# author-hidden-name/GAN-segmentation

Measured on AMD Instinct MI355X. Metric: synthetic (image,mask) pairs/sec, FFHQ-1024 StyleGAN+decoder, higher is better.
Workload: dtype f32; 1 GPU; stylegan-ffhq 1024^2 synthesis + 2-class decoder, batch=8 per GPU, fp32 (BASELINE.json configs[1]); synthetic weights/latents/noise; (img u8, mask u8) resident on rank 0; global_batch=8, parallelism=dp1, gather=none, backend=none, graph=eager (GSA_GRAPH=0)

## Files before the change

gan-segmentation_amd/csrc/gsa_api.cpp:

```cpp
#include <hip/hip_runtime.h>

#include <cmath>
#include <cstdarg>
#include <cstdio>
#include <cstdlib>
#include <cstring>
#include <map>
#include <string>
#include <vector>

#include "../../include/gsa.h"
#include "gsa_kernels.h"
#include "gsa_pack.h"

using namespace gsa;

namespace {

constexpr int kMaxLevels = 12;
thread_local std::string g_create_error;

struct HostTensor {
    std::vector<float> data;
    std::vector<int64_t> dims;
// ... 213 lines not shown
}

bool known_generator_name(const gsa_ctx* c, const char* name) {
    int R = 0, k = 0, i = 0;
    char tail[64], t2[64];
    if (!strcmp(name, "constant_tensor") || !strcmp(name, "latent_avg") || !strcmp(name, "truncation_psi")) return true;
    if (sscanf(name, "mp_dense_%d_%63s", &i, tail) == 2)
        return i >= 0 && i < 8 && (!strcmp(tail, "weight") || !strcmp(tail, "bias") || !strcmp(tail, "std"));
    if (sscanf(name, "%d_%63s", &R, tail) != 2) return false;
    int r = 0;
    while ((1 << r) < R) ++r;
    if ((1 << r) != R || r < 2 || r > c->gc.max_res_log2) return false;
    if (!strcmp(tail, "conv_1_weight") || !strcmp(tail, "conv_1_std")) return r > 2 && r < 7;
    if (!strcmp(tail, "deconv_1_weight") || !strcmp(tail, "deconv_1_std")) return r >= 7;
    if (!strcmp(tail, "blur_1_w_kernel")) return r > 2;
    if (!strcmp(tail, "conv_2_weight") || !strcmp(tail, "conv_2_std")) return true;
    if (!strcmp(tail, "conv_to_rgb_weight") || !strcmp(tail, "conv_to_rgb_bias") || !strcmp(tail, "conv_to_rgb_std"))
        return r == c->gc.max_res_log2;
    if (sscanf(tail, "noise_%d_%63s", &k, t2) == 2) return (k == 1 || k == 2) && !strcmp(t2, "scale_factors");
    if (sscanf(tail, "bias_%d_%63s", &k, t2) == 2) return (k == 1 || k == 2) && !strcmp(t2, "bias");
    if (sscanf(tail, "adain_%d_%63s", &k, t2) == 2)
        return (k == 1 || k == 2) &&
               (!strcmp(t2, "dense_affine_weight") || !strcmp(t2, "dense_affine_bias") || !strcmp(t2, "dense_affine_std") ||
                !strcmp(t2, "norm_gamma") || !strcmp(t2, "norm_beta"));
    return false;
}

int set_param(gsa_ctx* c, std::map<std::string, HostTensor>& m, const char* name, const float* data, int ndim,
              const int64_t* dims) {
    if (!name || !data || ndim < 0 || ndim > 8) return fail(c, GSA_ERR_INVALID, "bad parameter tensor %s", name ? name : "(null)");
    HostTensor t;
    size_t cnt = 1;
    for (int i = 0; i < ndim; ++i) {
        if (dims[i] < 0) return fail(c, GSA_ERR_INVALID, "negative dimension in %s", name);
        t.dims.push_back(dims[i]);
        cnt *= (size_t)dims[i];
    }
    t.data.assign(data, data + cnt);
    m[name] = std::move(t);
    return GSA_OK;
}


struct Launch {
    gsa_ctx* c;
    hipStream_t s;
    const char* label;
    double flops, bytes, alg;
    std::string entry_layer;
    hipEvent_t a = nullptr;
    Launch(gsa_ctx* ctx, hipStream_t st, const char* layer, double flops_, double bytes_, double alg_ = -1.0)
        : c(ctx), s(st), label(layer), flops(flops_), bytes(bytes_), alg(alg_ < 0 ? flops_ : alg_) {
        (void)take_launch_record();
        if (!c->prof) return;
        if (c->prof > 1 && layer) entry_layer = layer;
        if (c->bf16 && layer && strncmp(layer, "g.mapping", 9) && strncmp(layer, "g.styles", 8) && !strstr(layer, "finalize")) bytes *= 0.5;
        a = event();
        (void)hipEventRecord(a, s);
    }
    hipEvent_t event() {
        if (c->event_pool.empty()) {
            hipEvent_t e = nullptr;
            (void)hipEventCreate(&e);
            return e;
        }
        hipEvent_t e = c->event_pool.back();
        c->event_pool.pop_back();
        return e;
    }
    ~Launch() {
        const LaunchRecord r = take_launch_record();
#ifdef GSA_STAMP
        const std::string kname_s = r.count == 1 ? kernel_name(r.kern) : std::string();
        const char* kname = kname_s.c_str();
        if (c->stamps && label && (strstr(kname, "conv") || strstr(kname, "subpixel"))) {
            (void)hipStreamSynchronize(s);
            unsigned long long h[16];
            (void)hipMemcpy(h, c->stamps, sizeof h, hipMemcpyDeviceToHost);
            (void)hipMemset(c->stamps, 0, sizeof h);
            if (h[15] && strstr(kname, "_ws")) {
                const double w = (double)h[15];
                fprintf(stderr, "STAMPWS %-24s %-16s waves %6llu  mfma: work %9.0f barrier %9.0f | mem: write %9.0f load %9.0f epi %9.0f barrier %9.0f\n",
                        kname, label, h[15], h[0] / w, h[1] / w, h[2] / w, h[3] / w, h[4] / w, h[5] / w);
            } else if (h[15] && h[8]) {
                const double w = (double)h[12];
                fprintf(stderr, "STAMPDB %-70s %-14s waves %6llu items/wave %5.1f | per item: write %6.0f load %6.0f (epi-loads %5.0f index %5.0f bulk %5.0f) mfma %6.0f epi %6.0f barrier %6.0f\n",
                        kname, label, h[15], h[12] / (double)h[15], h[6] / w, h[7] / w, h[0] / w, h[1] / w, h[2] / w, h[8] / w, h[9] / w, h[10] / w);
                if (strstr(kname, "subpixel"))
                    fprintf(stderr, "STAMPSW %-14s barrier by wave: %6.0f %6.0f %6.0f %6.0f | write wave0 %6.0f wave3 %6.0f\n", label, 4 * h[0] / w, 4 * h[1] / w, 4 * h[2] / w, 4 * h[3] / w, 4 * h[4] / w, 4 * h[5] / w);
            } else if (h[15]) {
                const double w = (double)h[15];
                fprintf(stderr, "STAMP %-40s %-16s waves %8llu  load %7.0f  write %6.0f  bar %6.0f  blocks %8.0f  epi %7.0f\n", kname,
                        label, h[15], h[0] / w, h[1] / w, h[2] / w, h[3] / w, h[4] / w);
            }
        }
#endif
        if (!a) return;
        if (r.count != 1) {
            c->event_pool.push_back(a);
            if (r.count > 1) ++c->prof_multi;
            return;
        }
        int entry = -1;
        for (size_t i = 0; i < c->prof_entries.size() && entry < 0; ++i)
            if (c->prof_entries[i].kern == r.kern && c->prof_entries[i].layer == entry_layer) entry = (int)i;
        if (entry < 0) {
            ProfEntry e;
            e.kern = r.kern;
            e.layer = entry_layer;
            c->prof_entries.push_back(e);
            entry = (int)c->prof_entries.size() - 1;
        }
        ProfEntry& e = c->prof_entries[entry];
        e.flops += flops;
        e.alg_flops += alg;
        e.bytes += bytes;
        e.launches += 1;
        hipEvent_t b = event();
        (void)hipEventRecord(b, s);
        c->prof_events.push_back(ProfEvent{a, b, entry});
    }
};

}


extern "C" {

#define GSA_STR2(x) #x
#define GSA_STR(x) GSA_STR2(x)
const char* gsa_version(void) {
#ifndef GSA_EXPERIMENTS
#define GSA_EXPERIMENTS 0
#endif
    return "gsa-hip 0.5"
#if GSA_EXPERIMENTS
           "+experiments"
#endif
           " (gfx950, v_mfma_f32_16x16x4_f32 implicit-GEMM convs; built with hipcc = clang " __clang_version__
           ", HIP " GSA_STR(HIP_VERSION_MAJOR) "." GSA_STR(HIP_VERSION_MINOR) "." GSA_STR(HIP_VERSION_PATCH) ")";
}

int gsa_create(int device, gsa_ctx** out) {
    if (!out) return fail(nullptr, GSA_ERR_INVALID, "gsa_create: out is null");
    int count = 0;
    hipError_t e = hipGetDeviceCount(&count);
    if (e != hipSuccess || count <= 0)
        return fail(nullptr, GSA_ERR_HIP, "no HIP device available (%s)", e == hipSuccess ? "device count is 0" : hipGetErrorString(e));
    if (device < 0 || device >= count) return fail(nullptr, GSA_ERR_INVALID, "device %d out of range (%d devices)", device, count);
    e = hipSetDevice(device);
    if (e != hipSuccess) return fail(nullptr, GSA_ERR_HIP, "hipSetDevice(%d): %s", device, hipGetErrorString(e));
    gsa_ctx* c = new gsa_ctx();
    c->device = device;
    e = hipStreamCreateWithFlags(&c->side, hipStreamNonBlocking);
    for (int i = 0; e == hipSuccess && i < kMaxLevels; ++i) e = hipEventCreateWithFlags(&c->ev_level[i], hipEventDisableTiming);
    if (e == hipSuccess) e = hipEventCreateWithFlags(&c->ev_fork, hipEventDisableTiming);
    if (e == hipSuccess) e = hipEventCreateWithFlags(&c->ev_join, hipEventDisableTiming);
    if (e != hipSuccess) {
        const int rc = fail(nullptr, GSA_ERR_HIP, "creating the side stream: %s", hipGetErrorString(e));
        delete c;
        return rc;
    }
    if (e == hipSuccess) e = hipMalloc((void**)&c->zeros, 256);
    if (e == hipSuccess) e = hipMemset(c->zeros, 0, 256);
    if (e != hipSuccess) {
        const int rc = fail(nullptr, GSA_ERR_HIP, "allocating the zero page: %s", hipGetErrorString(e));
// ... 866 lines not shown
```

gan-segmentation_amd/csrc/gsa_kernels.hip:

```cpp
#include "gsa_kernels.h"
#include "gsa_dev.h"

#include <cxxabi.h>

#include <cstdio>
#include <cstdlib>
#include <cstring>
#include <mutex>
#include <vector>

#ifndef GSA_MFMA_PRIO
#define GSA_MFMA_PRIO 2
#endif
#ifndef GSA_OPERAND_PIPELINE
#define GSA_OPERAND_PIPELINE 1
#endif
#ifndef GSA_NO_XCD_REMAP
#define GSA_NO_XCD_REMAP 0
#endif
#ifndef GSA_POST_OCC
#define GSA_POST_OCC 2
#endif
#ifndef GSA_WINO_SOA
#define GSA_WINO_SOA 0
// ... 569 lines not shown
            TSUM(s0, k1, ka); TSUM(s1, ka, kb); TSUM(s2, kb, k2);
            mfma_item(it & 1, cb);
            TICK(k3);
            if (cb == nblk - 1) {
                epilogue(tc);
                if (stats_direct && (it + 1 >= total_items || tr.n != tc.n || tr.g != tc.g)) flush_stats(tc);
            }
            TICK(k4);
            write_aff_item(it & 1);
            __syncthreads();
            TICK(k5);
            TSUM(sw, k0, k1); TSUM(sl, k1, k2); TSUM(sm, k2, k3); TSUM(se, k3, k4); TSUM(sb, k4, k5);
            tc = tr; cb = cbr; tr = t2; cbr = cb2;
        }
        TFLUSH(6, sw); TFLUSH(7, sl); TFLUSH(8, sm); TFLUSH(9, se); TFLUSH(10, sb);
        TFLUSH(0, s0); TFLUSH(1, s1); TFLUSH(2, s2);
        TFLUSH(12, (unsigned long long)total_items); TFLUSH(15, 1ull);
        return;
    }

    WorkTile tc = decode(w_begin);
    TilePixel tp[AIT], tpn[AIT];
    tile_pixels(tc, tp);
    load_item(tc, 0, tp);
    int n_aff = tc.n;
    if (has_aff) {
        write_aff();
        __syncthreads();
    }
#ifdef GSA_STAMP
    asm volatile("s_waitcnt vmcnt(0)" ::: "memory");
#endif
    STAMP(1);
    write_item(0, tp, is_edge(tc));
    STAMP(2);
    __syncthreads();
    STAMP(3);

    int w = w_begin, cb = 0;
    while (true) {
        int w2 = w, cb2 = cb + 1;
        if (cb2 == nblk) { cb2 = 0; w2 = w + 1; }
        const bool has_next = w2 < w_end;
        if (!has_next) { w2 = w; cb2 = cb; }
        WorkTile tn = tc;
        if (w2 != w) {
            tn = advance(tc);
            tile_pixels(tn, tpn);
        } else {
#pragma unroll
            for (int it = 0; it < AIT; ++it) tpn[it] = tp[it];
        }
        load_item(tn, cb2, tpn);
        __builtin_amdgcn_sched_barrier(0);
        mfma_item(0);
        __builtin_amdgcn_sched_barrier(0);

        if (cb == nblk - 1) { epilogue_loads(tc); epilogue(tc); }
        if (!has_next) break;
        __syncthreads();
        if (has_aff && tn.n != n_aff) {
            write_aff();
            n_aff = tn.n;
            __syncthreads();
        }
#ifdef GSA_DBG_HOOKS
        if (!(p.dbg & 8))
#endif
        write_item(cb2, tpn, is_edge(tn));
        __syncthreads();
        tc = tn; w = w2; cb = cb2;
#pragma unroll
        for (int it = 0; it < AIT; ++it) tp[it] = tpn[it];
    }
    STAMP(4);
#ifdef GSA_STAMP
    asm volatile("s_waitcnt vmcnt(0)" ::: "memory");
#endif
    STAMP(5);
    STAMP_FLUSH(5);
}

__device__ __forceinline__ void finalize_one(const FinalizeParams& p, int n, int c, unsigned long long I1, unsigned long long I2);
template <int TH, int EPI, bool BF, int PS>
__global__ __launch_bounds__(256 * PS) void conv3x3_ksplit(ConvParams p) {
    constexpr int NTHR = 256 * PS, MT = (TH / 4) * (TH / 4), PW = TH / 4;
    constexpr int MTW = MT / PS;
    constexpr int LH = TH + 2, LW = TH + 2, NPX = LH * LW;
    constexpr int PX = BF ? 8 : 16, TS = BF ? 128 : 256, KQ = BF ? 2 : 4;
    constexpr int RS = LW * PX + (BF ? 4 : 8);
    constexpr int SEG = 9 * TS, IMG = LH * RS;
    constexpr int NB4 = 4 * SEG / 4, BIT = (NB4 + NTHR - 1) / NTHR;
    constexpr int QPT = PS == 1 ? 4 : 1;
    static_assert(PS == 1 || (PS == 2 && MT == 4 && 4 * NPX <= NTHR), "patch split: 8x8 tiles, one staged unit per thread");
    static_assert(NPX <= NTHR, "one staged pixel per thread and block");
    extern __shared__ __attribute__((aligned(16))) float smem[];
    float* sA = smem;
    float* sB = sA + 2 * 4 * IMG;
    f32x4* sAff = reinterpret_cast<f32x4*>(sB + 2 * 4 * SEG);
    f32x4* sP = sAff + 2 * 4 * 16;
    unsigned long long (*sfin)[16] = reinterpret_cast<unsigned long long (*)[16]>(sP + 4 * MT * 64);
    unsigned& sfin_cnt = *reinterpret_cast<unsigned*>(sfin + 2);
    if (EPI == EPI_SYNTH && p.fin_aff != nullptr && threadIdx.x < 33) {
        if (threadIdx.x < 32) sfin[threadIdx.x >> 4][threadIdx.x & 15] = 0ull; else sfin_cnt = 0u;
    }

    const int tid = threadIdx.x, lane = tid & 63;
    const int wave = __builtin_amdgcn_readfirstlane(tid >> 6);
    const int quarter = wave & 3, half = wave >> 2;
    const int i16 = lane & 15, kq = lane >> 4;
    const int tx = blockIdx.x % p.tiles_x, ty = blockIdx.x / p.tiles_x;
    const int g = blockIdx.y, n = blockIdx.z;
    const int y0 = ty * TH, x0 = tx * TH;
    const int nblk = p.C0 >> 4, nq = nblk >> 2;
    const bool has_aff = p.aff0 != nullptr;

    const int sq0 = PS == 1 ? 0 : tid / NPX;
    TilePixel tp;
    {
        const int st = PS == 1 ? tid : tid % NPX;
        const int ly = st / LW, lx = st % LW;
        const int gy = y0 + ly - 1, gx = x0 + lx - 1;
        const bool stage = PS == 1 ? tid < NPX : tid < 4 * NPX;
        const bool inside = stage && (unsigned)gy < (unsigned)p.H && (unsigned)gx < (unsigned)p.W;
        tp.lds = stage ? ly * RS + lx * PX : -1;
        tp.pix = inside ? (n * p.Hs + (gy >> p.up)) * p.Ws + (gx >> p.up) : -1;
    }
    int abase[MTW];
#pragma unroll
    for (int m = 0; m < MTW; ++m) {
        const int mt = half * MTW + m;
        abase[m] = ((mt / PW) * 4 + (i16 >> 2)) * RS + ((mt % PW) * 4 + (i16 & 3)) * PX + kq * KQ;
    }
    const int bbase = (kq * 16 + i16) * KQ;

    f32x4 acc[MTW];
#pragma unroll
    for (int m = 0; m < MTW; ++m) acc[m] = f32x4{0.f, 0.f, 0.f, 0.f};
    f32x4 ra[QPT][4], rb[BIT], rf;
    rf = f32x4{0.f, 0.f, 0.f, 0.f};
    const float* wgrp = p.wpk + (size_t)g * nblk * SEG;
    auto load_item = [&](int it) {
#pragma unroll
        for (int u = 0; u < QPT; ++u) load_pixel<BF>(ra[u], p.src0, p.C0, ((min(sq0, 3) + u) * nq + it) * 16, tp);
#pragma unroll
        for (int j = 0; j < BIT; ++j) {
            const int i = min(tid + j * NTHR, NB4 - 1);
            const int q = i / (SEG / 4), r = i % (SEG / 4);
            rb[j] = reinterpret_cast<const f32x4*>(wgrp + (size_t)(q * nq + it) * SEG)[r];
        }
        if (has_aff && tid < 64) rf = reinterpret_cast<const f32x4*>(p.aff0 + (size_t)n * p.C0 + ((tid >> 4) * nq + it) * 16)[tid & 15];
    };
    auto write_aff = [&](int buf) {
        if (has_aff && tid < 64) sAff[buf * 64 + tid] = rf;
    };
    auto write_item = [&](int buf) {
#pragma unroll
        for (int u = 0; u < QPT; ++u) {
            const int q = min(sq0, 3) + u;
            float* a_img = sA + (buf * 4 + q) * IMG;
            const float4* tab = reinterpret_cast<const float4*>(sAff) + (buf * 4 + q) * 16;
            if (has_aff) store_pixel<true, BF, true>(a_img, ra[u], tab, tp);
            else store_pixel<false, BF, true>(a_img, ra[u], tab, tp);
        }
#pragma unroll
        for (int j = 0; j < BIT; ++j) reinterpret_cast<f32x4*>(sB + buf * 4 * SEG)[min(tid + j * NTHR, NB4 - 1)] = rb[j];
    };
    auto mfma_item = [&](int buf) {
        const float* a_img = sA + (buf * 4 + quarter) * IMG;
        const float* b_img = sB + (buf * 4 + quarter) * SEG + bbase;
#pragma unroll
        for (int tap = 0; tap < 9; ++tap) {
            const int toff = (tap / 3) * RS + (tap % 3) * PX;
            if constexpr (BF) {
                const s16x4 b = *reinterpret_cast<const s16x4*>(b_img + tap * TS);
#pragma unroll
                for (int m = 0; m < MTW; ++m)
                    acc[m] = __builtin_amdgcn_mfma_f32_16x16x16bf16_1k(*reinterpret_cast<const s16x4*>(a_img + abase[m] + toff), b, acc[m], 0, 0, 0);
            } else {
                f32x4 a[MTW];
#pragma unroll
                for (int m = 0; m < MTW; ++m) a[m] = *reinterpret_cast<const f32x4*>(a_img + abase[m] + toff);
                const f32x4 b = *reinterpret_cast<const f32x4*>(b_img + tap * 256);
#pragma unroll
                for (int cg = 0; cg < 4; ++cg)
#pragma unroll
                    for (int m = 0; m < MTW; ++m) acc[m] = __builtin_amdgcn_mfma_f32_16x16x4f32(a[m][cg], b[cg], acc[m], 0, 0, 0);
            }
        }
    };

    load_item(0);
    write_aff(0);
    __syncthreads();
    write_item(0);
    load_item(min(1, nq - 1));
    write_aff(1);
    __syncthreads();
    unsigned long long k0 = 0, k1 = 0, k2 = 0, k3 = 0, k4 = 0, sw = 0, sl = 0, sm = 0, sb = 0;
    (void)k0; (void)k1; (void)k2; (void)k3; (void)k4; (void)sw; (void)sl; (void)sm; (void)sb;
    for (int it = 0; it < nq; ++it) {
        TICK(k0);
        if (it + 1 < nq) write_item((it + 1) & 1);
        TICK(k1);
        load_item(min(it + 2, nq - 1));
        TICK(k2);
        mfma_item(it & 1);
        TICK(k3);
        write_aff(it & 1);
        __syncthreads();
        TICK(k4);
        TSUM(sw, k0, k1); TSUM(sl, k1, k2); TSUM(sm, k2, k3); TSUM(sb, k3, k4);
    }
    TFLUSH(6, sw); TFLUSH(7, sl); TFLUSH(8, sm); TFLUSH(10, sb); TFLUSH(12, (unsigned long long)nq); TFLUSH(15, 1ull);
#pragma unroll
    for (int m = 0; m < MTW; ++m) sP[(quarter * MT + half * MTW + m) * 64 + lane] = acc[m];
    __syncthreads();
    if (wave >= MT) return;
    const int mt = wave;
    const f32x4 s01 = sP[(0 * MT + mt) * 64 + lane] + sP[(1 * MT + mt) * 64 + lane];
    const f32x4 s23 = sP[(2 * MT + mt) * 64 + lane] + sP[(3 * MT + mt) * 64 + lane];
    const f32x4 tot = s01 + s23;
    float v[4] = {tot[0], tot[1], tot[2], tot[3]};
    const int pr = mt / PW, pc = mt % PW, prow = lane >> 4;
    const int co = g * 16 + i16;
    const int y = y0 + pr * 4 + prow, xb = x0 + pc * 4;
    const int xj = lane & 3, cq4 = ((lane >> 2) & 3) * 4;
    if (EPI == EPI_SYNTH) {
        const float4 nz = *reinterpret_cast<const float4*>(p.noise + ((size_t)(n * p.H + y) * p.W + xb));
        const float nzv[4] = {nz.x, nz.y, nz.z, nz.w};
        const float e0 = p.nscale[co], e1 = p.nbias[co];
#pragma unroll
        for (int r = 0; r < 4; ++r) {
            const float t = e0 * nzv[r];
            v[r] = lrelu((v[r] + t) + e1);
        }
        const float sq = (v[0] + v[1]) + (v[2] + v[3]);
        const float qq = (v[0] * v[0] + v[1] * v[1]) + (v[2] * v[2] + v[3] * v[3]);
        unsigned long long I1 = to_fixed(sq, kStatScale1), I2 = to_fixed_sq(qq, stat_s2(p.H * p.W));
        I1 += shfl_xor_u64(I1, 16); I2 += shfl_xor_u64(I2, 16);
        I1 += shfl_xor_u64(I1, 32); I2 += shfl_xor_u64(I2, 32);
        if (p.fin_aff != nullptr) {
            if (lane < 16) { atomicAdd(&sfin[0][i16], I1); atomicAdd(&sfin[1][i16], I2); }
            __threadfence_block();
            unsigned arrived = 0;
            if (lane == 0) arrived = atomicAdd(&sfin_cnt, 1u);
            arrived = __shfl(arrived, 0);
            if (arrived == (unsigned)MT - 1u && lane < 16) {
                __threadfence_block();
                FinalizeParams f{};
                f.HW = p.H * p.W; f.C = p.Cout; f.style = p.fin_style; f.style_stride = p.fin_style_stride;
                f.gamma = p.fin_gamma; f.beta = p.fin_beta; f.aff = p.fin_aff; f.flags = p.fin_flags;
                finalize_one(f, n, co, atomicAdd(&sfin[0][i16], 0ull), atomicAdd(&sfin[1][i16], 0ull));
            }
        } else if (lane < 16) {
            StatPart sp; sp.s1 = I1; sp.s2 = I2;
            p.partials[((size_t)n * p.prow + blockIdx.x * MT + mt) * p.Cout + co] = sp;
        }
    }
    if (EPI == EPI_DEC) {
        const float e2 = p.bn_s[co], e3 = p.bn_beta[co];
#pragma unroll
        for (int r = 0; r < 4; ++r) {
            v[r] = lrelu(fmaf(v[r], e2, e3));
        }
    }
    f32x4 vt = quad_transpose(v[0], v[1], v[2], v[3], xj);
    if (EPI == EPI_DEC && p.resid != nullptr) {
        const int ru = p.resid_up;
        const size_t rpix = (size_t)(n * (p.H >> ru) + (y >> ru)) * (p.W >> ru) + ((xb + xj) >> ru);
        const int cch = g * 16;
        const bool second = p.resid1 != nullptr && cch >= p.res_c0;
        const int rcs = second ? p.Cout - p.res_c0 : (p.resid1 ? p.res_c0 : p.Cout);
        const f32x4 rr = act_load4<BF>((second ? p.resid1 : p.resid), rpix * rcs + (second ? cch - p.res_c0 : cch) + cq4);
#pragma unroll
        for (int r = 0; r < 4; ++r) vt[r] = rr[r] + vt[r];
    }
    act_store4<BF>(p.out, ((size_t)(n * p.H + y) * p.W + xb + xj) * p.Cout + g * 16 + cq4, vt);
}

template <int EPI, int NT, bool CHUNK, bool AFF, int GW = 1, int TW = 1>
__global__ __launch_bounds__(256 * GW * TW, NT == 1 ? 2 / TW : 1) void conv3x3_wino(ConvParams p) {
    static_assert(TW == 1 || (TW == 2 && GW == 1 && NT == 1), "two tiles per workgroup: one channel group, 16 output channels");
    constexpr int NTHR = 256 * GW * TW, LH = 18, LW = 16 * TW + 2, RS = LW * 16 + 4;
    constexpr int SEG = 16 * 256;
    constexpr int NB4 = SEG / 4, BIT = NT * NB4 / 256;
    constexpr int NCH = CHUNK ? (LH * LW * 4 + NTHR - 1) / NTHR : (LH * LW + NTHR - 1) / NTHR;
    constexpr int RW = CHUNK ? 1 : 4;
    extern __shared__ __attribute__((aligned(16))) float smem[];
    const int nblk = p.C0 >> 4;
    const bool wres = p.w_resident != 0;
    float* sA = smem;
    float* sB = sA + 2 * LH * RS;
    f32x4* sAff = reinterpret_cast<f32x4*>(sB + (wres ? nblk : 2) * GW * NT * SEG);

    const int tid = threadIdx.x, lane = tid & 63;
    const int wave8 = __builtin_amdgcn_readfirstlane(tid >> 6);
    const int wave = wave8 & 3;
    const int gsel = TW == 2 ? 0 : wave8 >> 2;
    const int tsel = TW == 2 ? wave8 >> 2 : 0;
    const int tid8 = tid & 255;
    const int i16 = lane & 15, kq = lane >> 4;
    int g, w_begin, w_end;
    if (p.group_minor) {
        const int b = blockIdx.x, j = b >> 3;
        g = (j % p.groups) * GW + gsel;
        w_begin = (j / p.groups) * 8 + (b & 7);
        w_end = w_begin + 1;
    } else {
        g = (int)blockIdx.y * GW + gsel;
        const int chunk = (p.total_tiles + (int)gridDim.x - 1) / (int)gridDim.x;
        w_begin = xcd_block(blockIdx.x, gridDim.x) * chunk;
        w_end = min(p.total_tiles, w_begin + chunk);
    }
    if (w_begin >= w_end) return;
    struct Tile { int n, y0, x0, row; };
    auto advance = [&](const Tile& t) {
        Tile u = t;
        u.x0 += 16 * TW; u.row += 1;
        if (u.x0 == p.W) { u.x0 = 0; u.y0 += 16; if (u.y0 == p.H) { u.y0 = 0; u.row = 0; u.n += 1; } }
        return u;
    };
    auto is_edge = [&](const Tile& t) { return t.y0 == 0 || t.x0 == 0 || t.y0 + 16 == p.H || t.x0 + 16 * TW == p.W; };
    const int part = tid & 3;
    int t_ly[NCH], t_lx[NCH], t_lds[NCH];
#pragma unroll
    for (int k = 0; k < NCH; ++k) {
        const int idx = CHUNK ? (tid + k * NTHR) >> 2 : tid + k * NTHR;
        t_ly[k] = idx / LW - 1; t_lx[k] = idx % LW - 1;
        t_lds[k] = idx < LH * LW ? (idx / LW) * RS + (idx % LW) * 16 + (CHUNK ? part * 4 : 0) : -1;
    }
    int t_rel[NCH];
#pragma unroll
    for (int k = 0; k < NCH; ++k) t_rel[k] = t_lds[k] >= 0 ? t_ly[k] * p.W + t_lx[k] : 0;
    auto tile_chunks = [&](const Tile& t, Chunk (&tp)[NCH]) {
        const int base = (t.n * p.H + t.y0) * p.W + t.x0;
        if (t.y0 == 0 || t.x0 == 0 || t.y0 + 16 == p.H || t.x0 + 16 * TW == p.W) {
#pragma unroll
            for (int k = 0; k < NCH; ++k) {
                const int gy = t.y0 + t_ly[k], gx = t.x0 + t_lx[k];
                const bool inside = t_lds[k] >= 0 && (unsigned)gy < (unsigned)p.H && (unsigned)gx < (unsigned)p.W;
                tp[k].lds = t_lds[k];
                tp[k].pix = inside ? base + t_rel[k] : -1;
            }
        } else {
#pragma unroll
            for (int k = 0; k < NCH; ++k) { tp[k].lds = t_lds[k]; tp[k].pix = base + t_rel[k]; }
        }
    };
    const int wty = ((i16 >> 3) & 1) * 2 + ((i16 >> 1) & 1), wtx = ((i16 >> 2) & 1) * 2 + (i16 & 1);
    const int pbase = ((wave >> 1) * 8 + 2 * wty) * RS + (tsel * 16 + (wave & 1) * 8 + 2 * wtx) * 16 + kq * 4;
    const int bbase = (kq * 16 + i16) * 4;

    f32x4 acc[16][NT];
#pragma unroll
    for (int f = 0; f < 16; ++f)
#pragma unroll
        for (int nt = 0; nt < NT; ++nt) acc[f][nt] = f32x4{0.f, 0.f, 0.f, 0.f};

    constexpr bool has_aff = AFF;
    constexpr bool kSoA = GSA_WINO_SOA != 0;
// ... 2417 lines not shown
    return enabled;
}

struct ConvGeom { int th, wm, wn, nt; };
static const ConvGeom kGeom4[] = {{4, 1, 4, 1}, {4, 1, 2, 1}, {4, 1, 1, 1}};
static const ConvGeom kGeom8[] = {{8, 4, 1, 4}, {8, 4, 1, 2}, {8, 4, 1, 1}};
static const ConvGeom kGeom16[] = {{16, 4, 1, 4}, {16, 4, 1, 2}, {16, 4, 1, 1}, {8, 4, 1, 4}, {8, 4, 1, 2}, {8, 4, 1, 1}};

static ConvGeom pick_geom(int H, int W, int Cout, int n) {
    const ConvGeom* cand = H == 4 ? kGeom4 : (H == 8 ? kGeom8 : kGeom16);
    const int ncand = H == 4 ? 3 : (H == 8 ? 3 : 6);
    ConvGeom best = cand[ncand - 1];
    long best_wgs = -1;
    for (int i = 0; i < ncand; ++i) {
        const ConvGeom& c = cand[i];
        const int ct = 16 * c.nt * c.wn;
        if (Cout % ct) continue;
        const long wgs = (long)(H / c.th) * (W / c.th) * (Cout / ct) * n;
        if (wgs >= 512) return c;
        if (wgs > best_wgs) { best_wgs = wgs; best = c; }
    }
    return best;
}

int conv_stat_rows(int H, int W, int Cout, int n) {
    const ConvGeom c = pick_geom(H, W, Cout, n);
    return (H / c.th) * (W / c.th) * c.wm;
}

int post_prow(int H, int W, int C) { return (H * (W / 4) * (C / 4) + 255) / 256; }

template <int TH, int TW, int WM, int WN, int NT, int EPI, bool SC, bool BF>
static hipError_t launch_conv_t(const ConvParams& p, int n, hipStream_t s) {
    constexpr int Q = NT * WN, COUT_T = 16 * Q;
    constexpr int TS = BF ? 128 : 256;
    constexpr int RS = (TW + 2) * (BF ? 8 : 16) + (BF ? 4 : 8);
    constexpr int NBUF = (Q <= 2 && !SC && (TH == 16 || GSA_DB_SMALL)) ? 2 : 1;
    const int nblk_all = (p.C0 + p.C1) / 16;
    static const bool wres_enabled = env_int("GSA_WRES", 1) != 0;
    const bool wres = wres_enabled && NBUF == 2 && p.Cout == COUT_T && (size_t)nblk_all * Q * 9 * TS * sizeof(float) <= 40 * 1024;
    if (NBUF == 1 && p.C0 > 512 && p.aff0) return hipErrorInvalidValue;
    const int wslots = wres ? nblk_all * Q * 9 * TS : NBUF * Q * 9 * TS;
    const size_t lds = sizeof(float) * (NBUF * (TH + 2) * RS + wslots + (SC ? Q * TS : 0)) +
                       (p.aff0 ? sizeof(float4) * (NBUF == 2 ? 32 : p.C0) : 0);
    constexpr auto kern = conv3x3_mfma<TH, TW, WM, WN, NT, EPI, SC, BF>;
    int wgs_per_cu = 0;
    if (hipError_t e = kernel_occupancy<kern>(p.device, 64 * WM * WN, lds, &wgs_per_cu)) return e;
    const int num_cus = device_cus(p.device);
    ConvParams q = p;
    q.w_resident = wres ? 1 : 0;
    q.tiles_x = p.W / TW;
    q.tiles_y = p.H / TH;
    q.groups = p.Cout / COUT_T;
    q.prow = q.tiles_x * q.tiles_y * WM;
    q.total_tiles = q.tiles_x * q.tiles_y * q.groups * n;
    const bool persistent = (p.C0 + p.C1) <= 32 && q.total_tiles > num_cus * wgs_per_cu;
    const int grid = persistent ? num_cus * wgs_per_cu : q.total_tiles;
    static const bool direct_enabled = env_int("GSA_STATS_DIRECT", 1) != 0;
    q.stats_direct = (direct_enabled && EPI == EPI_SYNTH && NBUF == 2 && persistent && p.partials != nullptr) ? 1 : 0;
    if (q.stats_direct) q.prow = kDirectRows;
    if (p.stat_rows_host) *p.stat_rows_host = q.prow;
    return launch<kern>(p.device, dim3(grid), dim3(64 * WM * WN), lds, s, q);
}

template <int TH, int TW, int WM, int WN, int NT>
static hipError_t launch_conv_g(const ConvParams& p, int epi, bool sc, int n, hipStream_t s) {
    if (sc && epi != EPI_DEC) return hipErrorInvalidValue;
#define GSA_EPI(BF) \
    if (sc) return launch_conv_t<TH, TW, WM, WN, NT, EPI_DEC, true, BF>(p, n, s); \
    if (epi == EPI_RAW) return launch_conv_t<TH, TW, WM, WN, NT, EPI_RAW, false, BF>(p, n, s); \
    if (epi == EPI_SYNTH) return launch_conv_t<TH, TW, WM, WN, NT, EPI_SYNTH, false, BF>(p, n, s); \
    if (epi == EPI_DEC) return launch_conv_t<TH, TW, WM, WN, NT, EPI_DEC, false, BF>(p, n, s); \
    return hipErrorInvalidValue;
    if (p.bf16) { GSA_EPI(true) }
    GSA_EPI(false)
#undef GSA_EPI
}

static bool ksplit_rule(const ConvParams& p, bool sc) {
    static const bool enabled = env_int("GSA_KSPLIT", 1) != 0;
    return enabled && !sc && p.src1 == nullptr && p.C1 == 0 && p.C0 >= 64 && p.C0 % 64 == 0 && (p.H <= 8 || (p.H <= 32 && p.Cout <= 32)) && p.H == p.W && p.Cout % 16 == 0;
}

template <int TH, int EPI, bool BF, int PS>
static hipError_t launch_ksplit_t(const ConvParams& p, int n, hipStream_t s) {
    constexpr int MT = (TH / 4) * (TH / 4), PX = BF ? 8 : 16, TS = BF ? 128 : 256;
    constexpr int RS = (TH + 2) * PX + (BF ? 4 : 8), IMG = (TH + 2) * RS, SEG = 9 * TS;
    const size_t lds = sizeof(float) * (2 * 4 * IMG + 2 * 4 * SEG) + sizeof(float4) * (2 * 4 * 16 + 4 * MT * 64) + 2 * 16 * sizeof(unsigned long long) + 16;
    ConvParams q = p;
    q.tiles_x = p.W / TH;
    q.tiles_y = p.H / TH;
    q.groups = p.Cout / 16;
    q.prow = q.tiles_x * q.tiles_y * MT;
    q.stats_direct = 0;
    if (p.stat_rows_host) *p.stat_rows_host = q.prow;
    return launch<conv3x3_ksplit<TH, EPI, BF, PS>>(p.device, dim3(q.tiles_x * q.tiles_y, q.groups, n), dim3(256 * PS), lds, s, q);
}

static int ksplit_ps() {
    static const int forced = env_int("GSA_KSPLIT_PS", 2);
    return forced == 1 ? 1 : 2;
}

static hipError_t launch_ksplit(const ConvParams& p, int epi, int n, hipStream_t s) {
#define GSA_KS(TH, BF, PS) \
    if ((p.H == 4 ? 4 : 8) == TH && (p.bf16 != 0) == BF && (TH == 4 ? 1 : ksplit_ps()) == PS) { \
        if (epi == EPI_RAW) return launch_ksplit_t<TH, EPI_RAW, BF, PS>(p, n, s); \
        if (epi == EPI_SYNTH) return launch_ksplit_t<TH, EPI_SYNTH, BF, PS>(p, n, s); \
        return launch_ksplit_t<TH, EPI_DEC, BF, PS>(p, n, s); \
    }
    GSA_KS(4, false, 1) GSA_KS(8, false, 1) GSA_KS(8, false, 2) GSA_KS(4, true, 1) GSA_KS(8, true, 1) GSA_KS(8, true, 2)
#undef GSA_KS
    return hipErrorInvalidValue;
}

static bool wino_rule(const ConvParams& p, int epi, bool sc) {
    static const bool enabled = env_int("GSA_WINO", 1) != 0;
    return enabled && p.wino != nullptr && !sc && !p.up && p.src1 == nullptr && p.C1 == 0 && epi != EPI_RAW &&
           wino_shape(p.H, p.Cout, p.bf16) && p.H == p.W && p.H % 16 == 0 && p.Cout % 16 == 0 && p.C0 % 16 == 0;
}

static int wino_nt(const ConvParams& p) {
    static const int forced = env_int("GSA_WINO_NT", 1);
    return (forced >= 2 && p.Cout % 32 == 0) ? 2 : 1;
}

template <int EPI, int NT, bool CHUNK, bool AFF, int GW, int TW = 1>
static hipError_t launch_wino_t(const ConvParams& p, int n, hipStream_t s) {
    constexpr int RS = (16 * TW + 2) * 16 + 4, SEG = 16 * 256;
    const int nblk = p.C0 / 16;
    const bool wres = (size_t)nblk * NT * SEG * sizeof(float) <= (NT == 1 ? 36 : 72) * 1024;
    const size_t lds = sizeof(float) * (2 * 18 * RS + (wres ? nblk : 2) * GW * NT * SEG) + (CHUNK ? 0 : 32 * sizeof(float4));
    constexpr auto kern = conv3x3_wino<EPI, NT, CHUNK, AFF, GW, TW>;
    if (TW == 2 && !wres) return hipErrorInvalidValue;
    int wgs_per_cu = 0;
    if (hipError_t e = kernel_occupancy<kern>(p.device, 256 * GW * TW, lds, &wgs_per_cu)) return e;
    const int num_cus = device_cus(p.device);
    ConvParams q = p;
    q.wpk = p.wino;
    q.w_resident = wres ? 1 : 0;
    q.tiles_x = p.W / (16 * TW);
    q.tiles_y = p.H / 16;
    q.groups = p.Cout / (16 * NT * GW);
    q.prow = q.tiles_x * q.tiles_y * 4 * TW;
    q.total_tiles = q.tiles_x * q.tiles_y * n;
    const int slots = std::max(1, num_cus * wgs_per_cu / q.groups);
    static const int pers_c = env_int("GSA_WINO_PERS", 1 << 30);
    const bool persistent = p.C0 <= pers_c && q.total_tiles > slots;
    const int gx = persistent ? slots : q.total_tiles;
    static const bool direct_enabled = env_int("GSA_STATS_DIRECT", 1) != 0;
    q.stats_direct = (direct_enabled && EPI == EPI_SYNTH && p.partials != nullptr && (persistent || (few_rows() && q.prow > kDirectRows))) ? 1 : 0;
    if (q.stats_direct) q.prow = kDirectRows;
    if (p.stat_rows_host) *p.stat_rows_host = q.prow;
    static const bool gm_enabled = env_int("GSA_WINO_GM", 1) != 0;
    q.group_minor = (gm_enabled && !persistent && q.groups > 1 && q.total_tiles % 8 == 0 &&
                     (size_t)16 * p.C0 * p.Cout * sizeof(float) <= (size_t)2 << 20) ? 1 : 0;
    const dim3 grid = q.group_minor ? dim3(q.total_tiles * q.groups) : dim3(gx, q.groups);
    return launch<kern>(p.device, grid, dim3(256 * GW * TW), lds, s, q);
}

#if GSA_EXPERIMENTS
bool wino43_enabled() {
    static const bool enabled = env_int("GSA_WINO43", 0) != 0;
    return enabled;
}

template <int EPI>
static hipError_t launch_wino43_t(const ConvParams& p, int n, hipStream_t s) {
    constexpr int IMG = 12 * 64 * 4, SEG = 36 * 128;
    const size_t lds = sizeof(float) * (4 * 2 * IMG + 2 * SEG);
    if (!p.zeros) return hipErrorInvalidValue;
    const int num_cus = device_cus(p.device);
    ConvParams q = p;
    q.wpk = p.wino;
    q.tiles_x = p.W / 16;
    q.tiles_y = p.H / 16;
    q.groups = p.Cout / 16;
    q.total_tiles = q.tiles_x * q.tiles_y * n;
    const int witems = (q.total_tiles + 3) / 4;
    const int slots = std::max(1, num_cus / q.groups);
    const int gx = std::min(witems, slots);
    q.stats_direct = 1;
    q.prow = kDirectRows;
    if (p.stat_rows_host) *p.stat_rows_host = q.prow;
    return launch<conv3x3_wino43<EPI>>(p.device, dim3(gx, q.groups), dim3(256), lds, s, q);
}

static hipError_t launch_wino43(const ConvParams& p, int epi, int n, hipStream_t s) {
    if (epi == EPI_SYNTH) return launch_wino43_t<EPI_SYNTH>(p, n, s);
    return launch_wino43_t<EPI_DEC>(p, n, s);
}

#else
bool wino43_enabled() { return false; }
// ... 411 lines not shown
```

Measured before the change: 1379 pairs/s.

## Interleave next-item LDS staging with MFMA taps in ksplit conv

Adds an 'ahead' variant of the k-split 3x3 conv kernel for fp32. It spreads the LDS writes and global loads for the next channel chunk across the nine MFMA taps, and double-buffers register operands per tap, so memory traffic overlaps with matrix math instead of running as a separate phase. For the 4x4 tile case it also rebalances activation staging so each wave stages one channel quarter. The variant is on by default through GSA_KSPLIT_AHEAD. It adds new stamp instrumentation and relies on sched_barrier ordering, which may raise register pressure.

```diff
diff --git a/gan-segmentation_amd/csrc/gsa_api.cpp b/gan-segmentation_amd/csrc/gsa_api.cpp
--- a/gan-segmentation_amd/csrc/gsa_api.cpp
+++ b/gan-segmentation_amd/csrc/gsa_api.cpp
@@ -319,6 +319,10 @@
                 const double w = (double)h[15];
                 fprintf(stderr, "STAMPWS %-24s %-16s waves %6llu  mfma: work %9.0f barrier %9.0f | mem: write %9.0f load %9.0f epi %9.0f barrier %9.0f\n",
                         kname, label, h[15], h[0] / w, h[1] / w, h[2] / w, h[3] / w, h[4] / w, h[5] / w);
+            } else if (h[15] && strstr(kname, "ksplit")) {
+                const double w = (double)h[12];
+                fprintf(stderr, "STAMPKS %-44s %-14s waves %6llu items/wave %4.1f | per item: wait %6.0f write %6.0f load-issue %6.0f mfma %6.0f barrier %6.0f | combine+epilogue %6.0f\n",
+                        kname, label, h[15], h[12] / (double)h[15], h[5] / w, h[6] / w, h[7] / w, h[8] / w, h[10] / w, h[11] ? h[9] / (double)h[11] : 0.0);
             } else if (h[15] && h[8]) {
                 const double w = (double)h[12];
                 fprintf(stderr, "STAMPDB %-70s %-14s waves %6llu items/wave %5.1f | per item: write %6.0f load %6.0f (epi-loads %5.0f index %5.0f bulk %5.0f) mfma %6.0f epi %6.0f barrier %6.0f\n",
diff --git a/gan-segmentation_amd/csrc/gsa_kernels.hip b/gan-segmentation_amd/csrc/gsa_kernels.hip
--- a/gan-segmentation_amd/csrc/gsa_kernels.hip
+++ b/gan-segmentation_amd/csrc/gsa_kernels.hip
@@ -675,8 +675,10 @@
 }
 
 __device__ __forceinline__ void finalize_one(const FinalizeParams& p, int n, int c, unsigned long long I1, unsigned long long I2);
-template <int TH, int EPI, bool BF, int PS>
+template <int TH, int EPI, bool BF, int PS, bool AH = false>
 __global__ __launch_bounds__(256 * PS) void conv3x3_ksplit(ConvParams p) {
+    static_assert(!AH || (!BF && ((TH == 4 && PS == 1) || PS == 2)), "interleaved staging: fp32, one staged unit per thread");
+    constexpr bool BAL = AH && PS == 1;
     constexpr int NTHR = 256 * PS, MT = (TH / 4) * (TH / 4), PW = TH / 4;
     constexpr int MTW = MT / PS;
     constexpr int LH = TH + 2, LW = TH + 2, NPX = LH * LW;
@@ -684,7 +686,7 @@
     constexpr int RS = LW * PX + (BF ? 4 : 8);
     constexpr int SEG = 9 * TS, IMG = LH * RS;
     constexpr int NB4 = 4 * SEG / 4, BIT = (NB4 + NTHR - 1) / NTHR;
-    constexpr int QPT = PS == 1 ? 4 : 1;
+    constexpr int QPT = PS == 1 && !BAL ? 4 : 1;
     static_assert(PS == 1 || (PS == 2 && MT == 4 && 4 * NPX <= NTHR), "patch split: 8x8 tiles, one staged unit per thread");
     static_assert(NPX <= NTHR, "one staged pixel per thread and block");
     extern __shared__ __attribute__((aligned(16))) float smem[];
@@ -708,13 +710,13 @@
     const int nblk = p.C0 >> 4, nq = nblk >> 2;
     const bool has_aff = p.aff0 != nullptr;
 
-    const int sq0 = PS == 1 ? 0 : tid / NPX;
+    const int sq0 = BAL ? tid >> 6 : PS == 1 ? 0 : tid / NPX;
     TilePixel tp;
     {
-        const int st = PS == 1 ? tid : tid % NPX;
+        const int st = BAL ? tid & 63 : PS == 1 ? tid : tid % NPX;
         const int ly = st / LW, lx = st % LW;
         const int gy = y0 + ly - 1, gx = x0 + lx - 1;
-        const bool stage = PS == 1 ? tid < NPX : tid < 4 * NPX;
+        const bool stage = BAL ? st < NPX : PS == 1 ? tid < NPX : tid < 4 * NPX;
         const bool inside = stage && (unsigned)gy < (unsigned)p.H && (unsigned)gx < (unsigned)p.W;
         tp.lds = stage ? ly * RS + lx * PX : -1;
         tp.pix = inside ? (n * p.Hs + (gy >> p.up)) * p.Ws + (gx >> p.up) : -1;
@@ -733,7 +735,11 @@
     f32x4 ra[QPT][4], rb[BIT], rf;
     rf = f32x4{0.f, 0.f, 0.f, 0.f};
     const float* wgrp = p.wpk + (size_t)g * nblk * SEG;
+    auto load_aff = [&](int it) {
+        if (has_aff && tid < 64) rf = reinterpret_cast<const f32x4*>(p.aff0 + (size_t)n * p.C0 + ((tid >> 4) * nq + it) * 16)[tid & 15];
+    };
     auto load_item = [&](int it) {
+        if (AH) load_aff(it);
 #pragma unroll
         for (int u = 0; u < QPT; ++u) load_pixel<BF>(ra[u], p.src0, p.C0, ((min(sq0, 3) + u) * nq + it) * 16, tp);
 #pragma unroll
@@ -742,7 +748,7 @@
             const int q = i / (SEG / 4), r = i % (SEG / 4);
             rb[j] = reinterpret_cast<const f32x4*>(wgrp + (size_t)(q * nq + it) * SEG)[r];
         }
-        if (has_aff && tid < 64) rf = reinterpret_cast<const f32x4*>(p.aff0 + (size_t)n * p.C0 + ((tid >> 4) * nq + it) * 16)[tid & 15];
+        if (!AH) load_aff(it);
     };
     auto write_aff = [&](int buf) {
         if (has_aff && tid < 64) sAff[buf * 64 + tid] = rf;
@@ -783,6 +789,30 @@
         }
     };
 
+    int wlds[AH ? BIT : 1], woff[AH ? BIT : 1];
+    if constexpr (AH) {
+#pragma unroll
+        for (int j = 0; j < BIT; ++j) {
+            const int i = min(tid + j * NTHR, NB4 - 1);
+            wlds[j] = i;
+            woff[j] = (i / (SEG / 4)) * nq * SEG + (i % (SEG / 4)) * 4;
+        }
+    }
+    auto stage_weight = [&](int nb, int j, int itl, bool live) {
+        reinterpret_cast<f32x4*>(sB + nb * 4 * SEG)[wlds[j]] = rb[j];
+        rb[j] = *reinterpret_cast<const f32x4*>(wgrp + (size_t)itl * SEG + (live ? woff[j] : 0));
+    };
+    auto stage_acts = [&](int nb, int itl) {
+        const int q = min(sq0, 3);
+        float* a_img = sA + (nb * 4 + q) * IMG;
+        const float4* tab = reinterpret_cast<const float4*>(sAff) + (nb * 4 + q) * 16;
+        if (has_aff) store_pixel<true, BF, true>(a_img, ra[0], tab, tp);
+        else store_pixel<false, BF, true>(a_img, ra[0], tab, tp);
+        load_pixel<BF>(ra[0], p.src0, p.C0, (q * nq + itl) * 16, tp);
+    };
+    (void)mfma_item; (void)stage_weight; (void)stage_acts;
+    unsigned long long k0 = 0, k1 = 0, k2 = 0, k3 = 0, k4 = 0, kw = 0, sv = 0, sw = 0, sl = 0, sm = 0, sb = 0;
+    (void)k0; (void)k1; (void)k2; (void)k3; (void)k4; (void)kw; (void)sv; (void)sw; (void)sl; (void)sm; (void)sb;
     load_item(0);
     write_aff(0);
     __syncthreads();
@@ -790,22 +820,64 @@
     load_item(min(1, nq - 1));
     write_aff(1);
     __syncthreads();
-    unsigned long long k0 = 0, k1 = 0, k2 = 0, k3 = 0, k4 = 0, sw = 0, sl = 0, sm = 0, sb = 0;
-    (void)k0; (void)k1; (void)k2; (void)k3; (void)k4; (void)sw; (void)sl; (void)sm; (void)sb;
-    for (int it = 0; it < nq; ++it) {
-        TICK(k0);
-        if (it + 1 < nq) write_item((it + 1) & 1);
-        TICK(k1);
-        load_item(min(it + 2, nq - 1));
-        TICK(k2);
-        mfma_item(it & 1);
-        TICK(k3);
-        write_aff(it & 1);
-        __syncthreads();
-        TICK(k4);
-        TSUM(sw, k0, k1); TSUM(sl, k1, k2); TSUM(sm, k2, k3); TSUM(sb, k3, k4);
-    }
-    TFLUSH(6, sw); TFLUSH(7, sl); TFLUSH(8, sm); TFLUSH(10, sb); TFLUSH(12, (unsigned long long)nq); TFLUSH(15, 1ull);
+    if constexpr (AH) {
+        for (int it = 0; it < nq; ++it) {
+            TICK(k0);
+            const int nb = (it + 1) & 1, itl = min(it + 2, nq - 1);
+            const bool live = it + 2 < nq;
+            load_aff(itl);
+            const float* a_img = sA + ((it & 1) * 4 + quarter) * IMG;
+            const float* b_img = sB + ((it & 1) * 4 + quarter) * SEG + bbase;
+            f32x4 a[2][MTW], b[2];
+#pragma unroll
+            for (int m = 0; m < MTW; ++m) a[0][m] = *reinterpret_cast<const f32x4*>(a_img + abase[m]);
+            b[0] = *reinterpret_cast<const f32x4*>(b_img);
+#pragma unroll
+            for (int tap = 0; tap < 9; ++tap) {
+                const int c = tap & 1;
+                if (tap + 1 < 9) {
+                    const int toff = ((tap + 1) / 3) * RS + ((tap + 1) % 3) * PX;
+#pragma unroll
+                    for (int m = 0; m < MTW; ++m) a[c ^ 1][m] = *reinterpret_cast<const f32x4*>(a_img + abase[m] + toff);
+                    b[c ^ 1] = *reinterpret_cast<const f32x4*>(b_img + (tap + 1) * 256);
+                }
+#pragma unroll
+                for (int cg = 0; cg < 4; ++cg)
+#pragma unroll
+                    for (int m = 0; m < MTW; ++m) acc[m] = __builtin_amdgcn_mfma_f32_16x16x4f32(a[c][m][cg], b[c][cg], acc[m], 0, 0, 0);
+#pragma unroll
+                for (int j = 0; j < BIT; ++j)
+                    if ((j * 9) / BIT == tap) stage_weight(nb, j, itl, live);
+                if (tap == 4) stage_acts(nb, itl);
+                __builtin_amdgcn_sched_barrier(0);
+            }
+            TICK(k3);
+            write_aff(it & 1);
+            __syncthreads();
+            TICK(k4);
+            TSUM(sm, k0, k3); TSUM(sb, k3, k4);
+        }
+    } else {
+        for (int it = 0; it < nq; ++it) {
+            TICK(k0);
+#ifdef GSA_STAMP
+            asm volatile("s_waitcnt vmcnt(0)" ::: "memory");
+#endif
+            TICK(kw);
+            if (it + 1 < nq) write_item((it + 1) & 1);
+            TICK(k1);
+            load_item(min(it + 2, nq - 1));
+            TICK(k2);
+            mfma_item(it & 1);
+            TICK(k3);
+            write_aff(it & 1);
+            __syncthreads();
+            TICK(k4);
+            TSUM(sv, k0, kw); TSUM(sw, kw, k1); TSUM(sl, k1, k2); TSUM(sm, k2, k3); TSUM(sb, k3, k4);
+        }
+    }
+#define GSA_KS_FLUSH() do { TFLUSH(5, sv); TFLUSH(6, sw); TFLUSH(7, sl); TFLUSH(8, sm); TFLUSH(10, sb); TFLUSH(12, (unsigned long long)nq); TFLUSH(15, 1ull); } while (0)
+    TICK(k0);
 #pragma unroll
     for (int m = 0; m < MTW; ++m) sP[(quarter * MT + half * MTW + m) * 64 + lane] = acc[m];
     __syncthreads();
@@ -870,6 +942,13 @@
         for (int r = 0; r < 4; ++r) vt[r] = rr[r] + vt[r];
     }
     act_store4<BF>(p.out, ((size_t)(n * p.H + y) * p.W + xb + xj) * p.Cout + g * 16 + cq4, vt);
+#ifdef GSA_STAMP
+    asm volatile("s_waitcnt vmcnt(0)" ::: "memory");
+#endif
+    TICK(k1);
+    GSA_KS_FLUSH();
+    TFLUSH(9, k1 - k0); TFLUSH(11, 1ull);
+#undef GSA_KS_FLUSH
 }
 
 template <int EPI, int NT, bool CHUNK, bool AFF, int GW = 1, int TW = 1>
@@ -3453,7 +3532,7 @@
     return enabled && !sc && p.src1 == nullptr && p.C1 == 0 && p.C0 >= 64 && p.C0 % 64 == 0 && (p.H <= 8 || (p.H <= 32 && p.Cout <= 32)) && p.H == p.W && p.Cout % 16 == 0;
 }
 
-template <int TH, int EPI, bool BF, int PS>
+template <int TH, int EPI, bool BF, int PS, bool AH = false>
 static hipError_t launch_ksplit_t(const ConvParams& p, int n, hipStream_t s) {
     constexpr int MT = (TH / 4) * (TH / 4), PX = BF ? 8 : 16, TS = BF ? 128 : 256;
     constexpr int RS = (TH + 2) * PX + (BF ? 4 : 8), IMG = (TH + 2) * RS, SEG = 9 * TS;
@@ -3465,7 +3544,7 @@
     q.prow = q.tiles_x * q.tiles_y * MT;
     q.stats_direct = 0;
     if (p.stat_rows_host) *p.stat_rows_host = q.prow;
-    return launch<conv3x3_ksplit<TH, EPI, BF, PS>>(p.device, dim3(q.tiles_x * q.tiles_y, q.groups, n), dim3(256 * PS), lds, s, q);
+    return launch<conv3x3_ksplit<TH, EPI, BF, PS, AH>>(p.device, dim3(q.tiles_x * q.tiles_y, q.groups, n), dim3(256 * PS), lds, s, q);
 }
 
 static int ksplit_ps() {
@@ -3473,14 +3552,20 @@
     return forced == 1 ? 1 : 2;
 }
 
+static bool ksplit_ahead() {
+    static const bool ahead = env_int("GSA_KSPLIT_AHEAD", 1) != 0;
+    return ahead;
+}
+
 static hipError_t launch_ksplit(const ConvParams& p, int epi, int n, hipStream_t s) {
-#define GSA_KS(TH, BF, PS) \
-    if ((p.H == 4 ? 4 : 8) == TH && (p.bf16 != 0) == BF && (TH == 4 ? 1 : ksplit_ps()) == PS) { \
-        if (epi == EPI_RAW) return launch_ksplit_t<TH, EPI_RAW, BF, PS>(p, n, s); \
-        if (epi == EPI_SYNTH) return launch_ksplit_t<TH, EPI_SYNTH, BF, PS>(p, n, s); \
-        return launch_ksplit_t<TH, EPI_DEC, BF, PS>(p, n, s); \
-    }
-    GSA_KS(4, false, 1) GSA_KS(8, false, 1) GSA_KS(8, false, 2) GSA_KS(4, true, 1) GSA_KS(8, true, 1) GSA_KS(8, true, 2)
+#define GSA_KS(TH, BF, PS, AH) \
+    if ((p.H == 4 ? 4 : 8) == TH && (p.bf16 != 0) == BF && (TH == 4 ? 1 : ksplit_ps()) == PS && (!BF && (TH == 4 || PS == 2) && ksplit_ahead()) == AH) { \
+        if (epi == EPI_RAW) return launch_ksplit_t<TH, EPI_RAW, BF, PS, AH>(p, n, s); \
+        if (epi == EPI_SYNTH) return launch_ksplit_t<TH, EPI_SYNTH, BF, PS, AH>(p, n, s); \
+        return launch_ksplit_t<TH, EPI_DEC, BF, PS, AH>(p, n, s); \
+    }
+    GSA_KS(4, false, 1, false) GSA_KS(4, false, 1, true) GSA_KS(8, false, 1, false) GSA_KS(8, false, 2, false) GSA_KS(8, false, 2, true)
+    GSA_KS(4, true, 1, false) GSA_KS(8, true, 1, false) GSA_KS(8, true, 2, false)
 #undef GSA_KS
     return hipErrorInvalidValue;
 }
```

New measurement: 1385 pairs/s (median of 6 runs). About the same (+0.4%).
